# zgojcic/3D_multiview_reg

Hardware: AMD Instinct MI355X
Metric: point-cloud pairs/s (feat+match+filter+SVD), 3DMatch 20k-pt, 1/2/4/8 GPU (higher is better)
Workload: dtype f32 (bf16x3 MFMA operands); 1 GPU; one synthetic 3DMatch-scale scene per GPU (configs[2]): 30 fragments x ~20393 voxels (0.025 m) -> FCGF -> rand 5000 samples -> soft feature-NN for all 435 pairs -> OANet (128ch, 500 clusters, 2 blocks) -> weighted Procrustes -> all-gather of (R,t,conf); sampler=rand, fragments_per_gpu=30, pairs_per_gpu=435, samples=5000, voxels_mean=20393, math=f32eq, oanet_point_layout=chunk-major, spconv_presplit_planes=False, spatial_map_order=False, library=e1fd863369cc629c, parallelism=dp1 (one scene per rank, RCCL all-gather of records)

## Files before the change

### 3d_multiview_reg_amd/csrc/knobs.hpp

```cpp
#pragma once

namespace mvr {

constexpr int GPU_CUS = 256;

extern int g_gemm_h;
extern int g_pconv_h;
extern int g_attn_h;
extern int g_spconv_h;
extern int g_feat_nn_fast;

enum ForcePath : int {
  FORCE_FEAT_NN_ONLINE = 0,
  FORCE_GENERIC_GEMM = 1,
  FORCE_UNFUSED_ATTN = 2,
  FORCE_NO_CONV1_FOLD = 3,
  FORCE_POOL_NOSPLIT = 4,
  FORCE_UNPOOL8 = 5,
  FORCE_ROW_LAYOUT = 6,
  FORCE_COUNT = 7
};
extern int g_force[FORCE_COUNT];

}
```

### 3d_multiview_reg_amd/csrc/spconv.hip

```cpp

#include "common.hpp"
#include "knobs.hpp"
#include "mfma_bf16.hpp"
#include "prof.hpp"
#include "sparse.hpp"

namespace mvr {

typedef float floatx16 __attribute__((ext_vector_type(16)));

struct SpArgs {
  const float* in; int64_t ldin; int Cin;
  const int32_t* nbr; int K; int64_t Mout;
  const int32_t* perm;
  const float* W; int Cout;
  const float* bias;
  mvr_bn_p bn; float bn_eps;
  const float* res; int64_t ldres;
  int relu;
  float* out; int64_t ldout;
  int* range; const int* guard; int epoch;
  const uint16_t* inp;
  uint16_t* outp;
};

constexpr int SP_KMAX = 32;
__device__ __attribute__((aligned(16))) float g_sp_zero[4];


#ifndef SP_TRACE
#define SP_TRACE 0
#endif
#if SP_TRACE
__device__ unsigned long long g_sp_trace[8];
#define SPSTAMP(slot)                                                  \
  do {                                                                 \
    unsigned long long t_;                                             \
    __builtin_amdgcn_sched_barrier(0);                                 \
    asm volatile("s_memtime %0\n\ts_waitcnt lgkmcnt(0)" : "=s"(t_));  \
    __builtin_amdgcn_sched_barrier(0);                                 \
    tr[prev_slot] += t_ - t_last;                                      \
    t_last = t_;                                                       \
    prev_slot = (slot);                                                \
  } while (0)
#else
#define SPSTAMP(slot) do {} while (0)
#endif

constexpr int SB_K = 32;
constexpr int SB_BST = 40;
constexpr int SB_CP = 128;
#ifndef SPBX_WBUF
#define SPBX_WBUF 1
#endif
#ifndef SPBX_NS32
#define SPBX_NS32 3
#endif
#ifndef SPBX_NS64
#define SPBX_NS64 3
#endif
#ifndef SPBX_NS128
#define SPBX_NS128 3
#endif
#ifndef SPBX_PS_NS32
#define SPBX_PS_NS32 3
#endif
#ifndef SPBX_PS_NS64
#define SPBX_PS_NS64 3
#endif
#ifndef SPBX_PS_NS128
#define SPBX_PS_NS128 2
#endif

template <int TN, int NS, int H, int PS>
__global__ __launch_bounds__(256, 2) void spconv_bx_kernel(SpArgs a, const uint16_t* __restrict__ wimg, int64_t CoutP,
                                                           const float* __restrict__ isc) {
  using namespace bx;
  constexpr int NPL = planes<H>();
  constexpr float XS = H ? 64.f : 1.f;
  constexpr int TM = 128;
  constexpr int NJ = TN / 32;
  constexpr int BPL = TN * SB_BST;
  constexpr int BG = NPL * BPL * 2 / 16;
  constexpr int GPT = (BG + 255) / 256;
  if (a.guard && *a.guard != a.epoch) return;
  __shared__ __attribute__((aligned(16))) uint16_t Bs[2][NPL * BPL];
  __shared__ int32_t nb[TM][SP_KMAX + 1];
  __shared__ int klist[SP_KMAX];
  __shared__ int orow_s[TM];
  __shared__ unsigned wmask[4];

  const int tid = threadIdx.x, lane = tid & 63, w = tid >> 6;
  const int l32 = lane & 31, h = lane >> 5;
#if SP_TRACE
  unsigned long long tr[8] = {0, 0, 0, 0, 0, 0, 0, 0}, t_last = __builtin_amdgcn_s_memtime();
  int prev_slot = 0;
#endif
  const int gy = (a.Cout + TN - 1) / TN;
  const int64_t t = (int64_t)blockIdx.x;
  const int64_t o0 = (t / gy) * TM;
  const int c0 = (int)(t % gy) * TN;
  const int K = a.K;

  if (tid < TM) {
    const int64_t o = o0 + tid;
    orow_s[tid] = o < a.Mout ? (int)(a.perm ? a.perm[o] : o) : -1;
  }
  __syncthreads();
  {
    constexpr int EMAX = (TM * SP_KMAX + 255) / 256;
    const int dq = 256 / K, dr = 256 - dq * K;
    int row = tid / K, k = tid - row * K;
    int vv[EMAX], ks[EMAX], rs[EMAX];
#pragma unroll
    for (int i = 0; i < EMAX; ++i) {
      ks[i] = k;
      rs[i] = row;
      vv[i] = -1;
      if (row < TM) {
        const int orow = orow_s[row];
        if (orow >= 0) vv[i] = a.nbr ? a.nbr[(int64_t)orow * K + k] : orow;
      }
      row += dq;
      k += dr;
      if (k >= K) {
        k -= K;
        ++row;
      }
    }
    unsigned m = 0;
#pragma unroll
    for (int i = 0; i < EMAX; ++i) {
      if (rs[i] < TM) {
        nb[rs[i]][ks[i]] = vv[i];
        if (vv[i] >= 0) m |= 1u << ks[i];
      }
    }
#pragma unroll
    for (int off = 32; off > 0; off >>= 1) m |= (unsigned)__shfl_xor((int)m, off, 64);
    if (lane == 0) wmask[w] = m;
  }
  __syncthreads();
  const unsigned kmask = wmask[0] | wmask[1] | wmask[2] | wmask[3];
  if (tid < K && ((kmask >> tid) & 1u)) klist[__popc(kmask & ((1u << tid) - 1u))] = tid;
  const int nk = __popc(kmask);
  __syncthreads();

  const int nci = (a.Cin + SB_K - 1) / SB_K;
  const int steps = nk * nci;
  const int row = 32 * w + l32;

  typedef float f32x4 __attribute__((ext_vector_type(4)));
  static_assert(!(PS && H), "pre-split planes are split-bf16");
  struct ASet {
    float4 v[PS ? 1 : 4];
    bf16x8 pv[PS ? 2 : 1][PS ? 3 : 1];
    f32x4 bq[GPT];
  };
  auto load_a = [&](int s, ASet& A) {
    if (s >= steps) s = steps - 1;
    const int k = klist[s / nci];
    const int ci0 = (s % nci) * SB_K;
    const int src = nb[row][k];
    if (PS) {
      const uint16_t* base = a.inp + (int64_t)(src >= 0 ? src : 0) * 3 * a.ldin;
#pragma unroll
      for (int st = 0; st < 2; ++st)
#pragma unroll
        for (int pl = 0; pl < 3; ++pl) {
          const uint16_t* pq = base + pl * a.ldin + ci0 + 16 * st + 8 * h;
          A.pv[st % (PS ? 2 : 1)][pl % (PS ? 3 : 1)] =
              *reinterpret_cast<const bf16x8*>(src >= 0 ? (const void*)pq : (const void*)g_sp_zero);
        }
    } else {
      const float* base = a.in + (int64_t)(src >= 0 ? src : 0) * a.ldin;
#pragma unroll
      for (int q = 0; q < 4; ++q) {
        const int ci = ci0 + 16 * (q >> 1) + 8 * h + 4 * (q & 1);
        const float* pq = src >= 0 ? base + ci : g_sp_zero;
        A.v[q % (PS ? 1 : 4)] = *reinterpret_cast<const float4*>(pq);
      }
    }
    const int cb = s % nci;
    const char* wb = reinterpret_cast<const char*>(wimg) + ((int64_t)(k * nci + cb) * NPL * CoutP + c0) * SB_BST * 2;
#if SPBX_WBUF
    const __amdgpu_buffer_rsrc_t rw = __builtin_amdgcn_make_buffer_rsrc(const_cast<char*>(wb), (short)0, 0x7fffffff,
                                                                        0x00020000);
#pragma unroll
    for (int i = 0; i < GPT; ++i) {
      const int g = min(tid + 256 * i, BG - 1);
      const int pl = g / (TN * 5), wi = g - pl * (TN * 5);
      A.bq[i] = __builtin_bit_cast(f32x4, __builtin_amdgcn_raw_buffer_load_b128(
                                              rw, pl * (int)CoutP * SB_BST * 2 + wi * 16, 0, 0));
    }
#else
#pragma unroll
    for (int i = 0; i < GPT; ++i) {
      const int g = min(tid + 256 * i, BG - 1);
      const int pl = g / (TN * 5), wi = g - pl * (TN * 5);
      A.bq[i] = *reinterpret_cast<const f32x4*>(wb + (int64_t)pl * CoutP * SB_BST * 2 + wi * 16);
    }
#endif
  };
  bool xbad = false;
  float xmx = 0.f;
  auto frag_a = [&](const ASet& A, int st) {
    if (PS) {
      FragT<H> f;
#pragma unroll
      for (int pl = 0; pl < planes<H>(); ++pl)
        f.p[pl] = __builtin_bit_cast(typename FragT<H>::V, A.pv[st % (PS ? 2 : 1)][pl % (PS ? 3 : 1)]);
      return f;
    }
    float v[8];
    const float4 x0 = A.v[(2 * st) % (PS ? 1 : 4)], x1 = A.v[(2 * st + 1) % (PS ? 1 : 4)];
    v[0] = x0.x; v[1] = x0.y; v[2] = x0.z; v[3] = x0.w;
    v[4] = x1.x; v[5] = x1.y; v[6] = x1.z; v[7] = x1.w;
    if (H) {
      float mx = 0.f;
#pragma unroll
      for (int i = 0; i < 8; ++i) {
        v[i] *= XS;
        mx = fmaxf(mx, fabsf(v[i]));
      }
      xbad |= !(mx < F16_RANGE);
      xmx = fmaxf(xmx, mx);
    }
    return split8t<H>(v);
  };
  auto store_b = [&](const ASet& A, int buf) {
    char* dst = reinterpret_cast<char*>(Bs[buf]);
#pragma unroll
    for (int i = 0; i < GPT; ++i) {
      const int g = tid + 256 * i;
      if (g < BG) *reinterpret_cast<f32x4*>(dst + g * 16) = A.bq[i];
    }
  };

  floatx16 acc[NJ];
#pragma unroll
  for (int j = 0; j < NJ; ++j)
#pragma unroll
    for (int r = 0; r < 16; ++r) acc[j][r] = 0.f;

  if (steps > 0) {
    ASet A[NS];
    SPSTAMP(7);
#pragma unroll
    for (int u = 0; u < NS; ++u) load_a(u, A[u]);
    store_b(A[0], 0);
    __syncthreads();
    auto step = [&](int s, ASet& A, const ASet& An) {
      const int cur = s & 1;
      SPSTAMP(1);
      if (s + 1 < steps) store_b(An, cur ^ 1);
      SPSTAMP(2);
      const FragT<H> fa0 = frag_a(A, 0), fa1 = frag_a(A, 1);
      SPSTAMP(3);
      load_a(s + NS, A);
      SPSTAMP(4);
      const uint16_t* Bq = Bs[cur];
#pragma unroll
      for (int st = 0; st < 2; ++st) {
        const FragT<H>& fa = st ? fa1 : fa0;
#pragma unroll
        for (int j = 0; j < NJ; ++j) {
          const uint16_t* bp = Bq + (32 * j + l32) * SB_BST + 16 * st + 8 * h;
          const FragT<H> fb = ld_frag<H>(reinterpret_cast<const char*>(bp), 2 * BPL);
          acc[j] = mma<H>(fa, fb, acc[j]);
        }
      }
      SPSTAMP(5);
      __syncthreads();
    };
    int s = 0;
    for (; s + NS - 1 < steps; s += NS) {
#pragma unroll
      for (int u = 0; u < NS; ++u) step(s + u, A[u], A[(u + 1) % NS]);
    }
#pragma unroll
    for (int u = 0; u < NS - 1; ++u)
      if (s + u < steps) step(s + u, A[u], A[(u + 1) % NS]);
  }

  SPSTAMP(6);
  int orr[16];
#pragma unroll
  for (int r = 0; r < 16; ++r) orr[r] = orow_s[32 * w + (r & 3) + 8 * (r >> 2) + 4 * h];
#pragma unroll
  for (int j = 0; j < NJ; ++j) {
    const int c = c0 + j * 32 + l32;
    if (c >= a.Cout) continue;
    float bsc = 1.f, bsh = 0.f;
    if (a.bn.gamma) {
      bsc = a.bn.gamma[c] / sqrtf(a.bn.var[c] + a.bn_eps);
      bsh = a.bn.beta[c] - a.bn.mean[c] * bsc;
    }
    const float bias = a.bias ? a.bias[c] : 0.f;
    const float is = H ? isc[c] : 1.f;
    float rv[16];
#pragma unroll
    for (int r = 0; r < 16; ++r) rv[r] = a.res && orr[r] >= 0 ? a.res[(int64_t)orr[r] * a.ldres + c] : 0.f;
#pragma unroll
    for (int r = 0; r < 16; ++r) {
      if (orr[r] < 0) continue;
      float v = (H ? acc[j][r] * is : acc[j][r]) + bias;
      v = fmaf(v, bsc, bsh);
      if (a.res) v += rv[r];
      if (a.relu) v = fmaxf(v, 0.f);
      a.out[(int64_t)orr[r] * a.ldout + c] = v;
      if (a.outp) bx::store_planes(a.outp + (int64_t)orr[r] * 3 * a.ldout + c, a.ldout, v);
    }
  }
  if (H && __any(xbad || (xmx > 0.f && xmx < 0.125f)) && lane == 0) atomicExch(a.range, a.epoch);
#if SP_TRACE
  SPSTAMP(0);
  if (lane == 0)
    for (int q = 0; q < 8; ++q) atomicAdd(&g_sp_trace[q], tr[q]);
#endif
}

__global__ void spconv_wscale_kernel(const float* __restrict__ W, int K, int Cin, int Cout, int64_t CoutP, float* wsc,
                                     float* isc) {
  const int64_t c = ((int64_t)blockIdx.x * blockDim.x + threadIdx.x) >> 6;
  const int lane = threadIdx.x & 63;
  if (c >= CoutP) return;
  float amax = 0.f;
  if (c < Cout)
    for (int64_t e = lane; e < (int64_t)K * Cin; e += 64) amax = fmaxf(amax, fabsf(W[e * Cout + c]));
#pragma unroll
  for (int o = 1; o < 64; o <<= 1) amax = fmaxf(amax, __shfl_xor(amax, o, 64));
  if (lane == 0) {
    const float s = bx::range_scale(amax);
    wsc[c] = s;
    isc[c] = 1.f / (s * 64.f);
  }
}

__global__ void spconv_wimage_kernel(const float* __restrict__ W, int K, int Cin, int Cout, int nci, int64_t CoutP,
                                     uint16_t* img, uint16_t* img16, const float* __restrict__ wsc) {
  using namespace bx;
  const int64_t e = (int64_t)blockIdx.x * blockDim.x + threadIdx.x;
  const int64_t total = (int64_t)K * nci * CoutP * 4;
  if (e >= total) return;
  const int q = (int)(e & 3);
  const int64_t t = e >> 2;
  const int c = (int)(t % CoutP);
  const int64_t kb = t / CoutP;
  const int cb = (int)(kb % nci), k = (int)(kb / nci);
  float v[8];
#pragma unroll
  for (int i = 0; i < 8; ++i) {
    const int ci = cb * SB_K + 8 * q + i;
    v[i] = (ci < Cin && c < Cout) ? W[((int64_t)k * Cin + ci) * Cout + c] : 0.f;
  }
  Frag f;
  split8(v, f.h, f.m, f.l);
  uint16_t* row = img + ((kb * 3) * CoutP + c) * SB_BST + 8 * q;
  *reinterpret_cast<bf16x8*>(row) = f.h;
  *reinterpret_cast<bf16x8*>(row + CoutP * SB_BST) = f.m;
  *reinterpret_cast<bf16x8*>(row + 2 * CoutP * SB_BST) = f.l;
  const float sc = wsc[c];
#pragma unroll
  for (int i = 0; i < 8; ++i) v[i] *= sc;
  const FragT<1> g = split8t<1>(v);
  uint16_t* row16 = img16 + ((kb * 2) * CoutP + c) * SB_BST + 8 * q;
  *reinterpret_cast<f16x8*>(row16) = g.p[0];
  *reinterpret_cast<f16x8*>(row16 + CoutP * SB_BST) = g.p[1];
}

#ifndef SPCONV_MATH_DEFAULT
#define SPCONV_MATH_DEFAULT 0
#endif
int g_spconv_h = SPCONV_MATH_DEFAULT;

}

using namespace mvr;

static int64_t sp_coutp(int Cout) { return ((int64_t)Cout + SB_CP - 1) / SB_CP * SB_CP; }

static size_t sp_bf16_bytes(int K, int Cin, int Cout) {
  return (size_t)K * ((Cin + SB_K - 1) / SB_K) * 3 * sp_coutp(Cout) * SB_BST * 2;
}
static size_t sp_f16_bytes(int K, int Cin, int Cout) { return sp_bf16_bytes(K, Cin, Cout) / 3 * 2; }

extern "C" size_t mvr_spconv_wimage_bytes(int K, int Cin, int Cout) {
  if (K <= 0 || Cin <= 0 || Cout <= 0) return 0;
  return sp_bf16_bytes(K, Cin, Cout) + sp_f16_bytes(K, Cin, Cout) + 2 * sp_coutp(Cout) * sizeof(float);
}

extern "C" int mvr_spconv_wimage(const float* W, int K, int Cin, int Cout, void* img, size_t bytes, hipStream_t s) {
  if (!W || !img || K <= 0 || K > SP_KMAX || Cin <= 0 || Cout <= 0 || bytes < mvr_spconv_wimage_bytes(K, Cin, Cout) ||
      (reinterpret_cast<uintptr_t>(img) & 15))
    return MVR_EINVAL;
  const int nci = (Cin + SB_K - 1) / SB_K;
  const int64_t CoutP = sp_coutp(Cout);
  const int64_t total = (int64_t)K * nci * CoutP * 4;
  char* base = reinterpret_cast<char*>(img);
  uint16_t* img16 = reinterpret_cast<uint16_t*>(base + sp_bf16_bytes(K, Cin, Cout));
  float* wsc = reinterpret_cast<float*>(base + sp_bf16_bytes(K, Cin, Cout) + sp_f16_bytes(K, Cin, Cout));
  hipLaunchKernelGGL(spconv_wscale_kernel, dim3((unsigned)((CoutP * 64 + 255) / 256)), dim3(256), 0, s, W, K, Cin, Cout,
                     CoutP, wsc, wsc + CoutP);
  MVR_CHECK_LAUNCH();
  hipLaunchKernelGGL(spconv_wimage_kernel, dim3((unsigned)((total + 255) / 256)), dim3(256), 0, s, W, K, Cin, Cout, nci,
                     CoutP, reinterpret_cast<uint16_t*>(img), img16, wsc);
  MVR_CHECK_LAUNCH();
  return MVR_OK;
}

extern "C" int mvr_spconv_x(const float* in, int64_t ldin, int Cin, const int32_t* nbr, const int32_t* perm, int K,
                            int64_t Mout, const float* W, int Cout, const float* bias, mvr_bn_p bn, float bn_eps,
                            const float* res, int64_t ldres, int relu, float* out, int64_t ldout, const void* wimg,
                            int32_t* range_flag, const uint16_t* in_planes, uint16_t* out_planes, hipStream_t s) {
  if (Cin <= 0 || Cout <= 0 || K <= 0 || K > SP_KMAX || Mout < 0) return MVR_EINVAL;
  if (Mout == 0) return MVR_OK;
  if (!in || !W || !out || !wimg) return MVR_EINVAL;
  if ((in_planes && ((ldin & 7) || (reinterpret_cast<uintptr_t>(in_planes) & 15))) ||
      (out_planes && (reinterpret_cast<uintptr_t>(out_planes) & 1)))
    return MVR_EINVAL;
  if (reinterpret_cast<uintptr_t>(wimg) & 15) return MVR_EINVAL;
  if (!nbr && K != 1) return MVR_EINVAL;
  if ((Cin % SB_K) || (Cout & 3) || (ldin & 3) || (reinterpret_cast<uintptr_t>(in) & 15) ||
      (reinterpret_cast<uintptr_t>(W) & 15))
    return MVR_EINVAL;
  SpArgs a{in, ldin, Cin, nbr, K, Mout, perm, W, Cout, bias, bn, bn_eps, res, ldres, relu, out, ldout,
           nullptr, nullptr, 0, in_planes, out_planes};
  ProfScope prof(PK_SPCONV, 2.0 * Mout * (double)K * Cin * Cout,
                 (double)Mout * (Cin + Cout) * 4.0 + (nbr ? (double)Mout * K * 4.0 : 0.0) + 4.0 * K * Cin * Cout, s);
  const char* base = reinterpret_cast<const char*>(wimg);
  const uint16_t* wi = reinterpret_cast<const uint16_t*>(wimg);
  const uint16_t* wi16 = reinterpret_cast<const uint16_t*>(base + sp_bf16_bytes(K, Cin, Cout));
  const int64_t CoutP = sp_coutp(Cout);
  const float* isc = reinterpret_cast<const float*>(base + sp_bf16_bytes(K, Cin, Cout) + sp_f16_bytes(K, Cin, Cout)) +
                     CoutP;
  const unsigned gx = (unsigned)((Mout + 127) / 128);
  const bool h1 = g_spconv_h && range_flag && Cout > 64 && res != out;
  if (h1) {
    if (hipMemsetAsync(range_flag, 0, sizeof(int32_t), s) != hipSuccess) return MVR_ELAUNCH;
    a.range = range_flag;
    a.epoch = 1;
  }
#define MVR_SPL(TN_, NS_, PNS_, GY)                                                                             \
  do {                                                                                                         \
    if (h1) {                                                                                                  \
      hipLaunchKernelGGL((spconv_bx_kernel<TN_, NS_, 1, 0>), dim3(gx * (GY)), dim3(256), 0, s, a, wi16, CoutP, isc); \
      MVR_CHECK_LAUNCH();                                                                                      \
      a.guard = a.range;                                                                                       \
      a.range = nullptr;                                                                                       \
    }                                                                                                          \
    if (in_planes)                                                                                             \
      hipLaunchKernelGGL((spconv_bx_kernel<TN_, PNS_, 0, 1>), dim3(gx * (GY)), dim3(256), 0, s, a, wi, CoutP, isc); \
    else                                                                                                       \
      hipLaunchKernelGGL((spconv_bx_kernel<TN_, NS_, 0, 0>), dim3(gx * (GY)), dim3(256), 0, s, a, wi, CoutP, isc); \
  } while (0)
  if (Cout <= 32)
    MVR_SPL(32, SPBX_NS32, SPBX_PS_NS32, 1);
  else if (Cout <= 64)
    MVR_SPL(64, SPBX_NS64, SPBX_PS_NS64, (Cout + 63) / 64);
  else
    MVR_SPL(128, SPBX_NS128, SPBX_PS_NS128, (Cout + 127) / 128);
#undef MVR_SPL
  MVR_CHECK_LAUNCH();
  return MVR_OK;
}

extern "C" int mvr_spconv(const float* in, int64_t ldin, int Cin, const int32_t* nbr, const int32_t* perm, int K,
                          int64_t Mout, const float* W, int Cout, const float* bias, mvr_bn_p bn, float bn_eps,
                          const float* res, int64_t ldres, int relu, float* out, int64_t ldout, const void* wimg,
                          int32_t* range_flag, hipStream_t s) {
  return mvr_spconv_x(in, ldin, Cin, nbr, perm, K, Mout, W, Cout, bias, bn, bn_eps, res, ldres, relu, out, ldout, wimg,
                      range_flag, nullptr, nullptr, s);
}

#if SP_TRACE
extern "C" int mvr_spconv_trace(unsigned long long* out, int reset) {
  if (hipMemcpyFromSymbol(out, HIP_SYMBOL(mvr::g_sp_trace), sizeof(unsigned long long) * 8) != hipSuccess) return -1;
  if (reset) {
    unsigned long long z[8] = {0, 0, 0, 0, 0, 0, 0, 0};
    if (hipMemcpyToSymbol(HIP_SYMBOL(mvr::g_sp_trace), z, sizeof(z)) != hipSuccess) return -1;
  }
  return 0;
}
#endif
```

### 3d_multiview_reg_amd/lib/_native.py

```python
import ctypes
import os

import torch

_PKG = os.path.dirname(os.path.dirname(os.path.abspath(__file__)))
LIB_PATH = os.environ.get("MVR_LIB") or os.path.join(_PKG, "libmvreg_hip.so")
_lib = None

c_i64 = ctypes.c_int64
c_int = ctypes.c_int
c_float = ctypes.c_float
c_vp = ctypes.c_void_p
c_size = ctypes.c_size_t


class ConvP(ctypes.Structure):
    _fields_ = [("weight", c_vp), ("bias", c_vp)]


class BnP(ctypes.Structure):
    _fields_ = [("gamma", c_vp), ("beta", c_vp), ("mean", c_vp), ("var", c_vp)]


class PointCNP(ctypes.Structure):
    _fields_ = [("bn1", BnP), ("conv3", ConvP), ("bn5", BnP), ("conv7", ConvP), ("shortcut", ConvP)]


class OAFilterP(ctypes.Structure):
    _fields_ = [("bn1", BnP), ("conv1", ConvP), ("bn2", BnP), ("conv2", ConvP), ("bn3", BnP), ("conv3", ConvP)]


MAX_HALF = 8


class OanBlockP(ctypes.Structure):
    _fields_ = [("in_channels", c_int), ("channels", c_int), ("clusters", c_int), ("half_layers", c_int),
                ("conv1", ConvP), ("l1_1", PointCNP * MAX_HALF), ("down_bn", BnP), ("down_conv", ConvP),
                ("l2", OAFilterP * MAX_HALF), ("up_bn", BnP), ("up_conv", ConvP), ("l1_2", PointCNP * MAX_HALF),
                ("output", ConvP)]


_SIGS = {
    "mvr_procrustes": (c_int, [c_vp, c_vp, c_i64, c_i64, c_vp, c_i64, c_vp, c_vp, c_i64, c_int, c_int, c_int, c_float,
                               c_vp, c_vp, c_vp, c_i64, c_vp, c_i64, c_vp, c_int, c_vp]),
    "mvr_procrustes_f64": (c_int, [c_vp, c_vp, c_i64, c_i64, c_vp, c_i64, c_vp, c_vp, c_i64, c_int, c_int, c_int,
                                   ctypes.c_double, c_vp, c_vp, c_vp, c_i64, c_vp, c_i64, c_vp, c_int, c_vp]),
    "mvr_ransac_workspace_bytes": (c_size, [c_int, c_int]),
    "mvr_ransac": (c_int, [c_vp, c_vp, c_i64, c_vp, c_int, c_int, c_int, ctypes.c_double, ctypes.c_uint64, c_vp, c_vp,
                           c_vp, c_vp, c_vp, c_vp, c_size, c_vp]),
    "mvr_ransac_checked_workspace_bytes": (c_size, [c_int, c_int, c_int]),
    "mvr_ransac_checked": (c_int, [c_vp, c_vp, c_i64, c_vp, c_int, c_int, c_int, ctypes.c_double, ctypes.c_uint64,
                                   c_int, ctypes.c_double, ctypes.c_double, c_vp, c_vp, ctypes.c_double, c_vp, c_vp,
                                   c_vp, c_vp, c_vp, c_vp, c_vp, c_vp, c_vp, c_vp, c_size, c_vp]),
    "mvr_fgr_workspace_bytes": (c_size, [c_int, c_int, c_int]),
    "mvr_fgr": (c_int, [c_vp, c_vp, c_i64, c_vp, c_int, ctypes.c_double, c_int, ctypes.c_double, c_int, c_int,
                        ctypes.c_double, ctypes.c_uint64, c_vp, c_vp, c_vp, c_vp, c_vp, c_vp, c_vp, c_vp, c_size,
                        c_vp]),
    "mvr_sync_workspace_bytes": (c_size, [c_int, c_int, c_int]),
    "mvr_sync_poses": (c_int, [c_vp, c_vp, c_vp, c_vp, c_i64, c_vp, c_vp, c_int, c_int, c_int, c_int, c_int,
                               ctypes.c_double, ctypes.c_double, c_vp, c_vp, c_i64, c_vp, c_vp, c_vp, c_vp, c_vp, c_vp,
                               c_size, c_vp]),
    "mvr_gemm_f32": (c_int, [c_int, c_int, c_int, c_int, c_vp, c_i64, c_i64, c_vp, c_i64, c_i64, c_int, c_vp, c_i64,
                             c_i64, c_vp, c_i64, c_vp, c_int, c_vp, c_vp, c_i64, c_i64, c_int, c_vp, c_i64, c_int,
                             c_int, c_int, c_vp, c_vp]),
    "mvr_oaf_conv2_f32": (c_int, [c_int, c_int, c_int, c_int, c_vp, c_i64, c_i64, c_vp, c_i64, c_vp, c_i64, c_i64,
                                  c_vp, c_i64, c_vp, c_vp, c_vp, c_i64, c_vp, c_i64, c_vp, c_i64, c_vp]),
    "mvr_oaf_conv2_image_bytes": (c_size, [c_int, c_int]),
    "mvr_oan_block_workspace_bytes": (c_size, [c_int, c_int, c_int, c_int, c_int]),
    "mvr_set_math": (c_int, [c_int]),
    "mvr_debug_force": (c_int, [c_int, c_int]),
    "mvr_attn_reruns": (c_int, [c_int]),
    "mvr_debug_stage_hash": (c_int, [c_vp, c_int]),
    "mvr_debug_stage_dump": (c_int, [c_int, c_vp, c_size]),
    "mvr_oan_diff_pool": (c_int, [c_vp, c_i64, c_i64, c_vp, c_vp, c_i64, c_vp, c_vp, c_int, c_int, c_int, c_int,
                                  c_vp, c_i64, c_i64, c_vp, c_i64, c_int, c_vp]),
    "mvr_oan_diff_pool_ws": (c_int, [c_vp, c_i64, c_i64, c_vp, c_vp, c_i64, c_vp, c_vp, c_int, c_int, c_int, c_int,
                                  c_vp, c_i64, c_i64, c_vp, c_i64, c_int, c_vp, c_size, c_vp]),
    "mvr_oan_diff_pool_workspace_bytes": (c_size, [c_int, c_int, c_int]),
    "mvr_oan_diff_unpool_workspace_bytes": (c_size, [c_int, c_int, c_int]),
    "mvr_oan_diff_unpool": (c_int, [c_vp, c_i64, c_i64, c_vp, c_vp, c_i64, c_vp, c_vp, c_vp, c_i64, c_i64, c_int,
                                    c_int, c_int, c_int, c_vp, c_i64, c_i64, c_vp, c_i64, c_int, c_vp, c_size, c_vp]),
    "mvr_oan_block_forward": (c_int, [ctypes.POINTER(OanBlockP), c_vp, c_i64, c_i64, c_vp, c_i64, c_i64, c_int, c_int, c_int,
                                      c_vp, c_vp, c_vp, c_vp, c_vp, c_vp, c_vp, c_vp, c_i64, c_vp, c_vp, c_int, c_vp,
                                      c_size, c_vp]),
    "mvr_feat_nn": (c_int, [c_vp, c_i64, c_vp, c_i64, c_vp, c_i64, c_vp, c_i64, c_vp, c_int, c_int, c_int, c_int,
                            c_float, c_int, c_vp, c_i64, c_i64, c_vp, c_vp]),
    "mvr_feat_nn_gumbel": (c_int, [c_vp, c_i64, c_vp, c_i64, c_vp, c_i64, c_vp, c_i64, c_vp, c_int, c_int, c_int,
                                   c_int, c_float, c_int, ctypes.c_uint64, c_vp, c_i64, c_i64, c_vp, c_vp]),
    "mvr_feat_nn_workspace_bytes": (c_size, [c_int, c_int]),
    "mvr_feat_nn_ws": (c_int, [c_vp, c_i64, c_vp, c_i64, c_vp, c_i64, c_vp, c_i64, c_vp, c_int, c_int, c_int, c_int,
                               c_float, c_int, c_vp, c_i64, c_i64, c_vp, c_int, c_vp, c_size, c_vp]),
    "mvr_gather_rows": (c_int, [c_vp, c_int, c_vp, c_int, c_vp, c_vp]),
    "mvr_sample_rand_mt19937": (c_int, [c_vp, c_vp, c_vp, c_int, c_int, c_vp, c_vp]),
    "mvr_feat_knn2": (c_int, [c_vp, c_i64, c_vp, c_i64, c_vp, c_int, c_int, c_int, c_int, c_vp, c_vp, c_vp]),
    "mvr_fps": (c_int, [c_vp, c_vp, c_vp, c_int, c_int, c_vp, c_vp]),
    "mvr_knn1": (c_int, [c_vp, c_i64, c_i64, c_vp, c_i64, c_i64, c_int, c_int, c_int, c_vp, c_vp, c_vp]),
    "mvr_mutuals": (c_int, [c_vp, c_i64, c_i64, c_vp, c_i64, c_i64, c_vp, c_i64, c_i64, c_vp, c_i64, c_i64, c_int,
                            c_int, c_float, c_vp, c_vp, c_vp]),
    "mvr_voxel_centroids_workspace_bytes": (c_size, [c_i64]),
    "mvr_voxel_centroids": (c_int, [c_vp, c_vp, c_int, c_i64, ctypes.c_double, c_vp, c_size, c_vp, c_vp, c_vp]),
    "mvr_voxel_centroids_colored": (c_int, [c_vp, c_vp, c_int, c_i64, ctypes.c_double, c_vp, c_size, c_vp, c_vp, c_vp,
                                            c_vp, c_vp]),
    "mvr_radius_index_bytes": (c_size, [c_i64]),
    "mvr_radius_index_build": (c_int, [c_vp, c_vp, c_int, c_i64, ctypes.c_double, c_vp, c_size, c_vp]),
    "mvr_radius_overlap_count": (c_int, [c_vp, c_size, c_vp, c_vp, c_int, c_i64, c_vp, c_vp, c_int, c_i64,
                                         ctypes.c_double, c_vp, c_vp]),
    "mvr_icp_refine": (c_int, [c_vp, c_size, c_vp, c_vp, c_int, c_i64, ctypes.c_double, c_vp, c_vp, c_int,
                               ctypes.c_double, c_int, ctypes.c_double, ctypes.c_double, c_vp, c_vp, c_vp, c_vp, c_vp,
                               c_vp, c_vp, c_vp]),
    "mvr_estimate_normals": (c_int, [c_vp, c_size, c_vp, c_vp, c_int, c_i64, ctypes.c_double, ctypes.c_double, c_vp,
                                     c_vp, c_vp, c_vp]),
    "mvr_icp_refine_plane": (c_int, [c_vp, c_size, c_vp, c_vp, c_vp, c_int, c_i64, ctypes.c_double, c_vp, c_vp, c_int,
                                     ctypes.c_double, c_int, ctypes.c_double, ctypes.c_double, c_vp, c_vp, c_vp, c_vp,
                                     c_vp, c_vp, c_vp, c_vp]),
    "mvr_icp_refine_generalized": (c_int, [c_vp, c_size, c_vp, c_vp, c_vp, c_int, c_i64, ctypes.c_double, c_vp, c_vp,
                                           c_int, ctypes.c_double, ctypes.c_double, c_int, ctypes.c_double,
                                           ctypes.c_double, c_vp, c_vp, c_vp, c_vp, c_vp, c_vp, c_vp, c_vp]),
    "mvr_icp_refine_robust": (c_int, [c_vp, c_size, c_vp, c_vp, c_vp, c_int, c_i64, ctypes.c_double, c_vp, c_vp,
                                      c_int, c_int, ctypes.c_double, ctypes.c_double, c_int, ctypes.c_double, c_int,
                                      ctypes.c_double, ctypes.c_double, c_vp, c_vp, c_vp, c_vp, c_vp, c_vp, c_vp, c_vp,
                                      c_vp]),
    "mvr_color_gradient": (c_int, [c_vp, c_size, c_vp, c_vp, c_vp, c_vp, c_int, c_i64, ctypes.c_double,
                                   ctypes.c_double, c_vp, c_vp, c_vp, c_vp]),
    "mvr_icp_refine_colored": (c_int, [c_vp, c_size, c_vp, c_vp, c_vp, c_vp, c_vp, c_int, c_i64, ctypes.c_double, c_vp,
                                       c_vp, c_int, ctypes.c_double, ctypes.c_double, c_int, ctypes.c_double, c_int,
                                       ctypes.c_double, ctypes.c_double, c_vp, c_vp, c_vp, c_vp, c_vp, c_vp, c_vp,
                                       c_vp, c_vp]),
    "mvr_pair_information": (c_int, [c_vp, c_size, c_vp, c_vp, c_int, c_i64, ctypes.c_double, c_vp, c_vp, c_int,
                                     ctypes.c_double, c_vp, c_vp, c_vp, c_vp, c_vp]),
    "mvr_compute_fpfh_workspace_bytes": (c_size, [c_i64]),
    "mvr_compute_fpfh": (c_int, [c_vp, c_size, c_vp, c_vp, c_vp, c_int, c_i64, ctypes.c_double, ctypes.c_double, c_vp,
                                 c_vp, c_vp, c_size, c_vp]),
    "mvr_knn_self_workspace_bytes": (c_size, [c_i64]),
    "mvr_knn_self": (c_int, [c_vp, c_size, c_vp, c_vp, c_int, c_i64, ctypes.c_double, c_int, c_vp, c_vp, c_vp, c_size,
                             c_vp]),
    "mvr_statistical_outlier": (c_int, [c_vp, c_vp, c_int, c_i64, c_int, ctypes.c_double, c_vp, c_vp, c_vp, c_vp]),
    "mvr_radius_count": (c_int, [c_vp, c_size, c_vp, c_vp, c_int, c_i64, ctypes.c_double, ctypes.c_double, c_vp,
                                 c_vp]),
    "mvr_iss_saliency": (c_int, [c_vp, c_size, c_vp, c_vp, c_int, c_i64, ctypes.c_double, ctypes.c_double,
                                 ctypes.c_double, ctypes.c_double, ctypes.c_double, c_int, c_vp, c_vp, c_vp]),
    "mvr_radius_nms": (c_int, [c_vp, c_size, c_vp, c_vp, c_int, c_i64, ctypes.c_double, ctypes.c_double, c_int, c_vp,
                               c_vp, c_vp]),
    "mvr_feat_match": (c_int, [c_vp, c_int, c_vp, c_int, c_i64, c_vp, c_vp, c_int, c_i64, c_i64, c_vp, c_vp, c_vp]),
    "mvr_posegraph_workspace_bytes": (c_size, [c_int, c_int, c_int]),
    "mvr_posegraph_optimize": (c_int, [c_vp, c_vp, c_vp, c_vp, c_vp, c_i64, c_vp, c_vp, c_int, c_int, c_int, c_int,
                                       c_vp, c_vp, c_int, ctypes.c_double, ctypes.c_double, ctypes.c_double, c_vp,
                                       c_vp, c_i64, c_vp, c_vp, c_vp, c_vp, c_vp, c_vp, c_size, c_vp]),
    "mvr_posegraph_lp_workspace_bytes": (c_size, [c_int, c_int, c_int]),
    "mvr_posegraph_optimize_lp": (c_int, [c_vp, c_vp, c_vp, c_vp, c_vp, c_vp, c_i64, c_vp, c_vp, c_int, c_int, c_int,
                                          c_int, c_vp, c_vp, c_int, ctypes.c_double, ctypes.c_double, ctypes.c_double,
                                          ctypes.c_double, c_vp, c_vp, c_i64, c_vp, c_vp, c_vp, c_vp, c_vp, c_vp, c_vp,
                                          c_vp, c_size, c_vp]),
    "mvr_fuse_scene_workspace_bytes": (c_size, [c_i64]),
    "mvr_fuse_scene": (c_int, [c_vp, c_vp, c_vp, c_int, c_i64, c_vp, c_vp, ctypes.c_double, c_vp, c_size, c_vp, c_vp,
                               c_vp, c_vp, c_vp, c_vp]),
    "mvr_hash_table_bytes": (c_size, [c_i64]),
    "mvr_voxelize_workspace_bytes": (c_size, [c_i64]),
    "mvr_voxelize_hint_workspace_bytes": (c_size, [c_i64, c_i64]),
    "mvr_voxelize_hint": (c_int, [c_vp, c_vp, c_int, c_i64, ctypes.c_double, c_i64, c_vp, c_size, c_vp, c_vp, c_vp,
                                  c_vp]),
    "mvr_voxelize": (c_int, [c_vp, c_vp, c_int, c_i64, ctypes.c_double, c_vp, c_size, c_vp, c_vp, c_vp, c_vp]),
    "mvr_voxelize_f64": (c_int, [c_vp, c_vp, c_int, c_i64, ctypes.c_double, c_vp, c_size, c_vp, c_vp, c_vp, c_vp]),
    "mvr_coords_downsample_workspace_bytes": (c_size, [c_i64]),
    "mvr_coords_downsample": (c_int, [c_vp, c_i64, c_int, c_int, c_vp, c_size, c_vp, c_vp, c_vp]),
    "mvr_hash_build": (c_int, [c_vp, c_i64, c_vp, c_size, c_vp]),
    "mvr_hash_build_lattice": (c_int, [c_vp, c_i64, c_int, c_vp, c_size, c_vp]),
    "mvr_kernel_map": (c_int, [c_vp, c_i64, c_vp, c_size, c_int, c_int, c_int, c_vp, c_vp]),
    "mvr_kernel_map_x": (c_int, [c_vp, c_i64, c_vp, c_size, c_int, c_int, c_int, c_vp, c_vp, c_vp]),
    "mvr_kernel_map_sym": (c_int, [c_vp, c_i64, c_vp, c_size, c_int, c_vp, c_vp]),
    "mvr_kernel_map_transpose": (c_int, [c_vp, c_i64, c_int, c_vp, c_i64, c_vp]),
    "mvr_kernel_map_order_bytes": (c_size, [c_i64]),
    "mvr_kernel_map_order": (c_int, [c_vp, c_vp, c_int, c_i64, c_int, c_vp, c_vp, c_size, c_vp]),
    "mvr_kernel_map_orders_bytes": (c_size, [c_i64]),
    "mvr_kernel_map_orders": (c_int, [c_int, c_vp, c_vp, c_vp, c_vp, c_int, c_vp, c_vp, c_size, c_vp]),
    "mvr_radix_sort_pairs_bytes": (c_size, [c_i64]),
    "mvr_radix_sort_pairs": (c_int, [c_vp, c_vp, c_i64, c_int, c_vp, c_vp, c_size, c_vp]),
    "mvr_spconv": (c_int, [c_vp, c_i64, c_int, c_vp, c_vp, c_int, c_i64, c_vp, c_int, c_vp, BnP, c_float, c_vp, c_i64,
                           c_int, c_vp, c_i64, c_vp, c_vp, c_vp]),
    "mvr_spconv_x": (c_int, [c_vp, c_i64, c_int, c_vp, c_vp, c_int, c_i64, c_vp, c_int, c_vp, BnP, c_float, c_vp,
                             c_i64, c_int, c_vp, c_i64, c_vp, c_vp, c_vp, c_vp, c_vp]),
    "mvr_spconv_c1_x": (c_int, [c_vp, c_i64, c_vp, c_i64, c_size, c_vp, c_int, c_int, c_vp, c_int, BnP, c_float,
                                c_int, c_vp, c_i64, c_vp, c_vp]),
    "mvr_spconv_wimage_bytes": (c_size, [c_int, c_int, c_int]),
    "mvr_spconv_wimage": (c_int, [c_vp, c_int, c_int, c_int, c_vp, c_size, c_vp]),
    "mvr_brick_map_bytes": (c_size, [c_i64]),
    "mvr_brick_map_build": (c_int, [c_vp, c_i64, c_vp, c_size, c_vp]),
    "mvr_brick_map_build_stride": (c_int, [c_vp, c_i64, c_int, c_vp, c_size, c_vp]),
    "mvr_spconv_c1": (c_int, [c_vp, c_i64, c_vp, c_i64, c_size, c_vp, c_int, c_int, c_vp, c_int, BnP, c_float, c_int,
                              c_vp, c_i64, c_vp]),
    "mvr_l2norm_rows": (c_int, [c_vp, c_i64, c_int, c_i64, c_vp]),
    "mvr_prof_set": (c_int, [c_int]),
    "mvr_prof_mask": (c_int, [ctypes.c_uint]),
    "mvr_prof_seq": (c_int, [c_vp, c_vp, c_int]),
    "mvr_prof_get": (c_int, [c_int, ctypes.POINTER(ctypes.c_double), ctypes.POINTER(ctypes.c_longlong),
                             ctypes.POINTER(ctypes.c_double), ctypes.POINTER(ctypes.c_double)]),
    "mvr_oan_last_layout": (c_int, []),
    "mvr_source_hash": (c_int, [ctypes.c_char_p, c_size]),
    "mvr_xs_to_channels": (c_int, [c_vp, c_i64, c_i64, c_int, c_int, c_int, c_vp, c_i64, c_i64, c_vp]),
}

EXPORTS = tuple(_SIGS)


def lib():
    global _lib
    if _lib is None:
        if not os.path.exists(LIB_PATH):
            raise RuntimeError("libmvreg_hip.so not found at %s — run __graft_entry__.build() "
                               "(there is no CPU fallback for the HIP path)" % LIB_PATH)
        L = ctypes.CDLL(LIB_PATH)
        for name, (res, args) in _SIGS.items():
            f = getattr(L, name)
            f.restype = res
            f.argtypes = args
        _lib = L
    return _lib


_hip_ok = False


def require_hip(t=None):
    global _hip_ok
    if not _hip_ok:
        if not torch.cuda.is_available():
            raise RuntimeError("mvreg HIP path: no HIP device available (no CPU fallback)")
        _hip_ok = True
    if t is not None and t.device.type != "cuda":
        raise RuntimeError("mvreg HIP path: tensor on %s, expected a HIP device" % t.device)


def stream():
    return c_vp(torch.cuda.current_stream().cuda_stream)


def ptr(t):
    if t is None:
        return None
    return c_vp(t.data_ptr())


def check(rc, name):
    if rc != 0:
        raise RuntimeError("%s failed with code %d" % (name, rc))


def hand_back(out, like, unbatch=False):
    if unbatch:
        out = {k: v[0] for k, v in out.items()}
    if not (torch.is_tensor(like) and like.device.type == "cuda"):
        out = {k: v.cpu() for k, v in out.items()}
        if not torch.is_tensor(like):
            out = {k: v.numpy() for k, v in out.items()}
    return out


def source_hash():
    buf = ctypes.create_string_buffer(128)
    check(lib().mvr_source_hash(buf, len(buf)), "mvr_source_hash")
    return buf.value.decode()


PROF_KINDS = {"conv_pts": 0, "embed": 1, "pool": 2, "unpool": 3, "oafilter": 4, "small": 5, "procrustes": 6,
              "feat_nn": 7, "spconv": 8, "sparse_misc": 9, "pointcn": 10}
RANSAC_CHECKED_PROF = {"check": 11, "scan": 12, "eval": 13, "select": 14}


def prof_set(on):
    check(lib().mvr_prof_set(int(on)), "mvr_prof_set")


def prof_mask(kinds=None):
    m = 0xFFFFFFFF if kinds is None else sum(1 << (PROF_KINDS[k] if isinstance(k, str) else int(k)) for k in kinds)
    check(lib().mvr_prof_mask(m), "mvr_prof_mask")


def prof_seq():
    import numpy as np
    L = lib()
    n = L.mvr_prof_seq(None, None, 0)
    k = np.zeros(max(n, 1), np.int32)
    b = np.zeros(max(n, 1), np.float64)
    L.mvr_prof_seq(k.ctypes.data, b.ctypes.data, n)
    names = {v: s for s, v in PROF_KINDS.items()}
    return [(names.get(int(k[i]), str(int(k[i]))), float(b[i])) for i in range(n)]


def prof_get(kind):
    ms, n, fl, by = ctypes.c_double(), ctypes.c_longlong(), ctypes.c_double(), ctypes.c_double()
    k = PROF_KINDS[kind] if isinstance(kind, str) else int(kind)
    check(lib().mvr_prof_get(k, ctypes.byref(ms), ctypes.byref(n), ctypes.byref(fl), ctypes.byref(by)),
          "mvr_prof_get")
    return ms.value, n.value, fl.value, by.value


MATH_KERNELS = "pconv_math,attn_math,spconv_math,gemm_f16,feat_nn"
FORCE = {"feat_nn_online": 0, "generic_gemm": 1, "unfused_attn": 2, "no_conv1_fold": 3, "pool_nosplit": 4,
         "unpool8": 5, "row_layout": 6}


def math_state():
    L = lib()
    m = L.mvr_set_math(0)
    L.mvr_set_math(m)
    return m


def set_math(mode):
    L = lib()
    L.mvr_set_math({"f32eq": 0, "split16": 1}[mode])
    m = math_state()
    dtype = "f32 (bf16x3 MFMA operands)" if not m else "mixed: split-fp16 (22-bit) operands in " + MATH_KERNELS
    return {"mode": "split16" if m else "f32eq", "dtype": dtype, "knobs": {"split16": m}}


class force:

    def __init__(self, what, value=1):
        self.what, self.value = FORCE[what], int(value)

    def __enter__(self):
        self.prev = lib().mvr_debug_force(self.what, self.value)
        return self

    def __exit__(self, *a):
        lib().mvr_debug_force(self.what, self.prev)


_ws_cache = {}
_flag_cache = {}


def flag_word(device=None):
    idx = (device.index if device is not None and device.index is not None else torch.cuda.current_device())
    key = (idx, torch.cuda.current_stream(idx).cuda_stream)
    buf = _flag_cache.get(key)
    if buf is None:
        buf = torch.zeros(64, dtype=torch.int32, device=torch.device("cuda", idx))
        _flag_cache[key] = buf
    return buf


def workspace(nbytes, device):
    idx = device.index if device.index is not None else torch.cuda.current_device()
    key = (idx, torch.cuda.current_stream(idx).cuda_stream)
    buf = _ws_cache.get(key)
    if buf is None or buf.numel() < nbytes:
        buf = torch.empty(max(int(nbytes), 1), dtype=torch.uint8, device=device)
        _ws_cache[key] = buf
    if _WS_POISON:
        buf[:int(nbytes)].fill_(0x7F)
    return buf


_WS_POISON = os.environ.get("MVR_WS_POISON") == "1"
```

Before: 10900 pairs/s.

## Stage spconv weight tiles into LDS via dedicated DMA loader waves

Adds a warp-specialized variant of the sparse-conv kernel in which extra loader waves copy pre-tiled weight stages directly from global memory into LDS with global-to-LDS loads, using a multi-slot ring synchronised by vmcnt waits and barriers. The compute waves no longer load B into registers and store it to shared memory. A new contiguous per-tile weight image is written during weight preparation so each stage is one linear copy. It is enabled by default only for the 128-channel tile case and only when the grid is at most one block per CU. The cost is larger blocks, more LDS slots, lower occupancy bounds and extra weight-image memory.

```diff
diff --git a/3d_multiview_reg_amd/csrc/knobs.hpp b/3d_multiview_reg_amd/csrc/knobs.hpp
--- a/3d_multiview_reg_amd/csrc/knobs.hpp
+++ b/3d_multiview_reg_amd/csrc/knobs.hpp
@@ -18,7 +18,8 @@
   FORCE_POOL_NOSPLIT = 4,
   FORCE_UNPOOL8 = 5,
   FORCE_ROW_LAYOUT = 6,
-  FORCE_COUNT = 7
+  FORCE_SPCONV_REGSTAGE = 7,
+  FORCE_COUNT = 8
 };
 extern int g_force[FORCE_COUNT];
 
diff --git a/3d_multiview_reg_amd/csrc/spconv.hip b/3d_multiview_reg_amd/csrc/spconv.hip
--- a/3d_multiview_reg_amd/csrc/spconv.hip
+++ b/3d_multiview_reg_amd/csrc/spconv.hip
@@ -72,10 +72,64 @@
 #define SPBX_PS_NS128 2
 #endif
 
-template <int TN, int NS, int H, int PS>
-__global__ __launch_bounds__(256, 2) void spconv_bx_kernel(SpArgs a, const uint16_t* __restrict__ wimg, int64_t CoutP,
-                                                           const float* __restrict__ isc) {
+#ifndef SPBX_DMA32
+#define SPBX_DMA32 0
+#endif
+#ifndef SPBX_DMA64
+#define SPBX_DMA64 0
+#endif
+#ifndef SPBX_DMA128
+#define SPBX_DMA128 1
+#endif
+#ifndef SPBX_DMA_GRID
+#define SPBX_DMA_GRID GPU_CUS
+#endif
+#ifndef SPBX_DSL32
+#define SPBX_DSL32 3
+#endif
+#ifndef SPBX_DSL64
+#define SPBX_DSL64 2
+#endif
+#ifndef SPBX_DSL128
+#define SPBX_DSL128 2
+#endif
+#ifndef SPBX_DNS32
+#define SPBX_DNS32 3
+#endif
+#ifndef SPBX_DNS64
+#define SPBX_DNS64 3
+#endif
+#ifndef SPBX_DNS128
+#define SPBX_DNS128 3
+#endif
+#ifndef SPBX_DOCC32
+#define SPBX_DOCC32 4
+#endif
+#ifndef SPBX_DOCC64
+#define SPBX_DOCC64 3
+#endif
+#ifndef SPBX_DOCC128
+#define SPBX_DOCC128 2
+#endif
+#ifndef SPBX_DLW32
+#define SPBX_DLW32 1
+#endif
+#ifndef SPBX_DLW64
+#define SPBX_DLW64 1
+#endif
+#ifndef SPBX_DLW128
+#define SPBX_DLW128 2
+#endif
+constexpr int sp_dma_waves(int TN) { return TN == 32 ? SPBX_DLW32 : TN == 64 ? SPBX_DLW64 : SPBX_DLW128; }
+constexpr int sp_dma_occ(int TN) { return TN == 32 ? SPBX_DOCC32 : TN == 64 ? SPBX_DOCC64 : SPBX_DOCC128; }
+constexpr int sp_dma_slots(int TN) { return TN == 32 ? SPBX_DSL32 : TN == 64 ? SPBX_DSL64 : SPBX_DSL128; }
+constexpr int sp_stage_bytes(int TN) { return 3 * TN * SB_BST * 2; }
+
+template <int TN, int NS, int H, int PS, int D = 0>
+__global__ __launch_bounds__(D ? 256 + 64 * sp_dma_waves(TN) : 256, D ? sp_dma_occ(TN) : 2) void spconv_bx_kernel(
+    SpArgs a, const uint16_t* __restrict__ wimg, int64_t CoutP, const float* __restrict__ isc) {
   using namespace bx;
+  static_assert(!D || (!H && !PS), "the DMA-staged form is split-bf16 on fp32 gathers");
   constexpr int NPL = planes<H>();
   constexpr float XS = H ? 64.f : 1.f;
   constexpr int TM = 128;
@@ -84,7 +138,14 @@
   constexpr int BG = NPL * BPL * 2 / 16;
   constexpr int GPT = (BG + 255) / 256;
   if (a.guard && *a.guard != a.epoch) return;
-  __shared__ __attribute__((aligned(16))) uint16_t Bs[2][NPL * BPL];
+  constexpr int SL = D ? sp_dma_slots(TN) : 2;
+  constexpr int STB = NPL * BPL * 2;
+  constexpr int NP = (STB + 1023) / 1024;
+  static_assert(SL == 2 || SL == 3, "stage slots");
+  constexpr int LW = sp_dma_waves(TN);
+  static_assert(NP % LW == 0, "whole pieces per loader wave");
+  static_assert((SL - 2) * NP / LW < 64, "vmcnt is 6 bits");
+  __shared__ __attribute__((aligned(16))) uint16_t Bs[SL][NPL * BPL];
   __shared__ int32_t nb[TM][SP_KMAX + 1];
   __shared__ int klist[SP_KMAX];
   __shared__ int orow_s[TM];
@@ -92,6 +153,7 @@
 
   const int tid = threadIdx.x, lane = tid & 63, w = tid >> 6;
   const int l32 = lane & 31, h = lane >> 5;
+  const int wu = D ? __builtin_amdgcn_readfirstlane(tid >> 6) : 0;
 #if SP_TRACE
   unsigned long long tr[8] = {0, 0, 0, 0, 0, 0, 0, 0}, t_last = __builtin_amdgcn_s_memtime();
   int prev_slot = 0;
@@ -107,7 +169,7 @@
     orow_s[tid] = o < a.Mout ? (int)(a.perm ? a.perm[o] : o) : -1;
   }
   __syncthreads();
-  {
+  if (!D || wu < 4) {
     constexpr int EMAX = (TM * SP_KMAX + 255) / 256;
     const int dq = 256 / K, dr = 256 - dq * K;
     int row = tid / K, k = tid - row * K;
@@ -148,6 +210,43 @@
 
   const int nci = (a.Cin + SB_K - 1) / SB_K;
   const int steps = nk * nci;
+
+  if (D && wu >= 4) {
+    if (steps > 0) {
+      const char* tiled = reinterpret_cast<const char*>(wimg);
+      const uint32_t bs0 = lds_addr(&Bs[0][0]);
+      auto dma_b = [&](int s) {
+        const int k = klist[s / nci];
+        const int blk = __builtin_amdgcn_readfirstlane((k * nci + s % nci) * gy + (int)(t % gy));
+        const char* src = tiled + (int64_t)blk * STB;
+        const uint32_t dst = bs0 + (uint32_t)((s % SL) * STB);
+#pragma unroll
+        for (int q = 0; q < NP / LW; ++q) {
+          const int p = LW * q + (LW > 1 ? wu - 4 : 0);
+          if ((LW * q + LW) * 1024 <= STB || lane * 16 < STB - p * 1024)
+            glds16s(src, (uint32_t)(p * 1024 + lane * 16), dst + (uint32_t)(p * 1024));
+        }
+      };
+#pragma unroll
+      for (int u = 0; u < SL - 1; ++u)
+        if (u < steps) dma_b(u);
+      if (steps >= SL - 1)
+        asm volatile("s_waitcnt vmcnt(%0)" ::"n"((SL - 2) * NP / LW) : "memory");
+      else
+        asm volatile("s_waitcnt vmcnt(0)" ::: "memory");
+      __syncthreads();
+      for (int s = 0; s < steps; ++s) {
+        if (s + SL - 1 < steps) {
+          dma_b(s + SL - 1);
+          asm volatile("s_waitcnt vmcnt(%0)" ::"n"((SL - 2) * NP / LW) : "memory");
+        } else {
+          asm volatile("s_waitcnt vmcnt(0)" ::: "memory");
+        }
+        __syncthreads();
+      }
+    }
+    return;
+  }
   const int row = 32 * w + l32;
 
   typedef float f32x4 __attribute__((ext_vector_type(4)));
@@ -155,7 +254,7 @@
   struct ASet {
     float4 v[PS ? 1 : 4];
     bf16x8 pv[PS ? 2 : 1][PS ? 3 : 1];
-    f32x4 bq[GPT];
+    f32x4 bq[D ? 1 : GPT];
   };
   auto load_a = [&](int s, ASet& A) {
     if (s >= steps) s = steps - 1;
@@ -181,6 +280,7 @@
         A.v[q % (PS ? 1 : 4)] = *reinterpret_cast<const float4*>(pq);
       }
     }
+    if (D) return;
     const int cb = s % nci;
     const char* wb = reinterpret_cast<const char*>(wimg) + ((int64_t)(k * nci + cb) * NPL * CoutP + c0) * SB_BST * 2;
 #if SPBX_WBUF
@@ -190,7 +290,7 @@
     for (int i = 0; i < GPT; ++i) {
       const int g = min(tid + 256 * i, BG - 1);
       const int pl = g / (TN * 5), wi = g - pl * (TN * 5);
-      A.bq[i] = __builtin_bit_cast(f32x4, __builtin_amdgcn_raw_buffer_load_b128(
+      A.bq[i % (D ? 1 : GPT)] = __builtin_bit_cast(f32x4, __builtin_amdgcn_raw_buffer_load_b128(
                                               rw, pl * (int)CoutP * SB_BST * 2 + wi * 16, 0, 0));
     }
 #else
@@ -198,7 +298,7 @@
     for (int i = 0; i < GPT; ++i) {
       const int g = min(tid + 256 * i, BG - 1);
       const int pl = g / (TN * 5), wi = g - pl * (TN * 5);
-      A.bq[i] = *reinterpret_cast<const f32x4*>(wb + (int64_t)pl * CoutP * SB_BST * 2 + wi * 16);
+      A.bq[i % (D ? 1 : GPT)] = *reinterpret_cast<const f32x4*>(wb + (int64_t)pl * CoutP * SB_BST * 2 + wi * 16);
     }
 #endif
   };
@@ -233,7 +333,7 @@
 #pragma unroll
     for (int i = 0; i < GPT; ++i) {
       const int g = tid + 256 * i;
-      if (g < BG) *reinterpret_cast<f32x4*>(dst + g * 16) = A.bq[i];
+      if (g < BG) *reinterpret_cast<f32x4*>(dst + g * 16) = A.bq[i % (D ? 1 : GPT)];
     }
   };
 
@@ -248,12 +348,12 @@
     SPSTAMP(7);
 #pragma unroll
     for (int u = 0; u < NS; ++u) load_a(u, A[u]);
-    store_b(A[0], 0);
+    if (!D) store_b(A[0], 0);
     __syncthreads();
     auto step = [&](int s, ASet& A, const ASet& An) {
-      const int cur = s & 1;
+      const int cur = D ? s % SL : s & 1;
       SPSTAMP(1);
-      if (s + 1 < steps) store_b(An, cur ^ 1);
+      if (!D && s + 1 < steps) store_b(An, cur ^ 1);
       SPSTAMP(2);
       const FragT<H> fa0 = frag_a(A, 0), fa1 = frag_a(A, 1);
       SPSTAMP(3);
@@ -338,7 +438,8 @@
 }
 
 __global__ void spconv_wimage_kernel(const float* __restrict__ W, int K, int Cin, int Cout, int nci, int64_t CoutP,
-                                     uint16_t* img, uint16_t* img16, const float* __restrict__ wsc) {
+                                     uint16_t* img, uint16_t* img16, const float* __restrict__ wsc, uint16_t* tiled,
+                                     int TNL, int gy) {
   using namespace bx;
   const int64_t e = (int64_t)blockIdx.x * blockDim.x + threadIdx.x;
   const int64_t total = (int64_t)K * nci * CoutP * 4;
@@ -360,6 +461,13 @@
   *reinterpret_cast<bf16x8*>(row) = f.h;
   *reinterpret_cast<bf16x8*>(row + CoutP * SB_BST) = f.m;
   *reinterpret_cast<bf16x8*>(row + 2 * CoutP * SB_BST) = f.l;
+  if (c < gy * TNL) {
+    const int ct = c / TNL, cl = c - ct * TNL;
+    uint16_t* tr = tiled + (((kb * gy + ct) * 3) * TNL + cl) * SB_BST + 8 * q;
+    *reinterpret_cast<bf16x8*>(tr) = f.h;
+    *reinterpret_cast<bf16x8*>(tr + TNL * SB_BST) = f.m;
+    *reinterpret_cast<bf16x8*>(tr + 2 * TNL * SB_BST) = f.l;
+  }
   const float sc = wsc[c];
 #pragma unroll
   for (int i = 0; i < 8; ++i) v[i] *= sc;
@@ -380,14 +488,24 @@
 
 static int64_t sp_coutp(int Cout) { return ((int64_t)Cout + SB_CP - 1) / SB_CP * SB_CP; }
 
+static int sp_tn(int Cout) { return Cout <= 32 ? 32 : Cout <= 64 ? 64 : 128; }
+
 static size_t sp_bf16_bytes(int K, int Cin, int Cout) {
   return (size_t)K * ((Cin + SB_K - 1) / SB_K) * 3 * sp_coutp(Cout) * SB_BST * 2;
 }
 static size_t sp_f16_bytes(int K, int Cin, int Cout) { return sp_bf16_bytes(K, Cin, Cout) / 3 * 2; }
 
+static size_t sp_tiled_off(int K, int Cin, int Cout) {
+  return sp_bf16_bytes(K, Cin, Cout) + sp_f16_bytes(K, Cin, Cout) + 2 * sp_coutp(Cout) * sizeof(float);
+}
+static size_t sp_tiled_bytes(int K, int Cin, int Cout) {
+  const int TN = sp_tn(Cout);
+  return (size_t)K * ((Cin + SB_K - 1) / SB_K) * ((Cout + TN - 1) / TN) * sp_stage_bytes(TN);
+}
+
 extern "C" size_t mvr_spconv_wimage_bytes(int K, int Cin, int Cout) {
   if (K <= 0 || Cin <= 0 || Cout <= 0) return 0;
-  return sp_bf16_bytes(K, Cin, Cout) + sp_f16_bytes(K, Cin, Cout) + 2 * sp_coutp(Cout) * sizeof(float);
+  return sp_tiled_off(K, Cin, Cout) + sp_tiled_bytes(K, Cin, Cout);
 }
 
 extern "C" int mvr_spconv_wimage(const float* W, int K, int Cin, int Cout, void* img, size_t bytes, hipStream_t s) {
@@ -403,8 +521,12 @@
   hipLaunchKernelGGL(spconv_wscale_kernel, dim3((unsigned)((CoutP * 64 + 255) / 256)), dim3(256), 0, s, W, K, Cin, Cout,
                      CoutP, wsc, wsc + CoutP);
   MVR_CHECK_LAUNCH();
+  const int TN = sp_tn(Cout);
+  char* tiled = base + sp_tiled_off(K, Cin, Cout);
+  if (hipMemsetAsync(tiled, 0, sp_tiled_bytes(K, Cin, Cout), s) != hipSuccess) return MVR_ELAUNCH;
   hipLaunchKernelGGL(spconv_wimage_kernel, dim3((unsigned)((total + 255) / 256)), dim3(256), 0, s, W, K, Cin, Cout, nci,
-                     CoutP, reinterpret_cast<uint16_t*>(img), img16, wsc);
+                     CoutP, reinterpret_cast<uint16_t*>(img), img16, wsc, reinterpret_cast<uint16_t*>(tiled), TN,
+                     (Cout + TN - 1) / TN);
   MVR_CHECK_LAUNCH();
   return MVR_OK;
 }
@@ -431,6 +553,7 @@
   const char* base = reinterpret_cast<const char*>(wimg);
   const uint16_t* wi = reinterpret_cast<const uint16_t*>(wimg);
   const uint16_t* wi16 = reinterpret_cast<const uint16_t*>(base + sp_bf16_bytes(K, Cin, Cout));
+  const uint16_t* wit = reinterpret_cast<const uint16_t*>(base + sp_tiled_off(K, Cin, Cout));
   const int64_t CoutP = sp_coutp(Cout);
   const float* isc = reinterpret_cast<const float*>(base + sp_bf16_bytes(K, Cin, Cout) + sp_f16_bytes(K, Cin, Cout)) +
                      CoutP;
@@ -441,7 +564,7 @@
     a.range = range_flag;
     a.epoch = 1;
   }
-#define MVR_SPL(TN_, NS_, PNS_, GY)                                                                             \
+#define MVR_SPL(TN_, NS_, PNS_, GY, DMA_, DNS_)                                                                          \
   do {                                                                                                         \
     if (h1) {                                                                                                  \
       hipLaunchKernelGGL((spconv_bx_kernel<TN_, NS_, 1, 0>), dim3(gx * (GY)), dim3(256), 0, s, a, wi16, CoutP, isc); \
@@ -451,15 +574,19 @@
     }                                                                                                          \
     if (in_planes)                                                                                             \
       hipLaunchKernelGGL((spconv_bx_kernel<TN_, PNS_, 0, 1>), dim3(gx * (GY)), dim3(256), 0, s, a, wi, CoutP, isc); \
-    else                                                                                                       \
+    else if ((DMA_) && !g_force[FORCE_SPCONV_REGSTAGE] && (!SPBX_DMA_GRID || (int64_t)gx * (GY) <= SPBX_DMA_GRID))  \
+      hipLaunchKernelGGL((spconv_bx_kernel<TN_, (DMA_) ? DNS_ : NS_, 0, 0, (DMA_) ? 1 : 0>), dim3(gx * (GY)),   \
+                         dim3((DMA_) ? 256 + 64 * sp_dma_waves(TN_) : 256), 0, s, a, (DMA_) ? wit : wi, CoutP, \
+                         isc);                                                                                 \
+    else                                                                                                      \
       hipLaunchKernelGGL((spconv_bx_kernel<TN_, NS_, 0, 0>), dim3(gx * (GY)), dim3(256), 0, s, a, wi, CoutP, isc); \
   } while (0)
   if (Cout <= 32)
-    MVR_SPL(32, SPBX_NS32, SPBX_PS_NS32, 1);
+    MVR_SPL(32, SPBX_NS32, SPBX_PS_NS32, 1, SPBX_DMA32, SPBX_DNS32);
   else if (Cout <= 64)
-    MVR_SPL(64, SPBX_NS64, SPBX_PS_NS64, (Cout + 63) / 64);
+    MVR_SPL(64, SPBX_NS64, SPBX_PS_NS64, (Cout + 63) / 64, SPBX_DMA64, SPBX_DNS64);
   else
-    MVR_SPL(128, SPBX_NS128, SPBX_PS_NS128, (Cout + 127) / 128);
+    MVR_SPL(128, SPBX_NS128, SPBX_PS_NS128, (Cout + 127) / 128, SPBX_DMA128, SPBX_DNS128);
 #undef MVR_SPL
   MVR_CHECK_LAUNCH();
   return MVR_OK;
diff --git a/3d_multiview_reg_amd/lib/_native.py b/3d_multiview_reg_amd/lib/_native.py
--- a/3d_multiview_reg_amd/lib/_native.py
+++ b/3d_multiview_reg_amd/lib/_native.py
@@ -296,7 +296,7 @@
 
 MATH_KERNELS = "pconv_math,attn_math,spconv_math,gemm_f16,feat_nn"
 FORCE = {"feat_nn_online": 0, "generic_gemm": 1, "unfused_attn": 2, "no_conv1_fold": 3, "pool_nosplit": 4,
-         "unpool8": 5, "row_layout": 6}
+         "unpool8": 5, "row_layout": 6, "spconv_regstage": 7}
 
 
 def math_state():
```

Result: no change. 10910 pairs/s (median of 6 runs) (+0.1%).
